# jizongFox/MI-based-Regularized-Semi-supervised-Segmentation

Measured on AMD Instinct MI355X. Metric: images/sec (UNet+IIC fwd/bwd) ACDC 256^2, higher is better.
Workload: dtype bf16; 1 GPU; udaiic train step, ACDC-shaped 1x256x256 4-class slices, LB=UB=16 per GPU, taps Conv5/Up_conv3/Up_conv2, K=20 x 5 sub-heads, paddings [1,3] (BASELINE configs[1]); mi_precision=f16f8, global_batch=32, parallelism=dp1, launch_tape=True, tape_ops=170, tape_replays_in_run=449

## Files before the change

### include/miseg_hip.h

```cpp
#ifndef MISEG_HIP_H
#define MISEG_HIP_H

#include <stdint.h>

#ifdef __cplusplus
extern "C" {
#endif

#define MISEG_F32 0
#define MISEG_BF16 1
#define MISEG_F16 2

#define MISEG_OK 0
#define MISEG_E_INVALID (-1)
#define MISEG_E_LAUNCH (-2)

int miseg_version(void);
const char* miseg_last_error(void);
int miseg_stream_wait_stream(void* waiter, void* producer);

int64_t miseg_tape_begin(void);
int miseg_tape_end(int64_t tape);
int miseg_tape_free(int64_t tape);
int64_t miseg_tape_mark(int64_t tape);
// ... 194 lines not shown
int miseg_bn_relu_fwd_acc(void* stream, int dt, const void* raw, int64_t N, int64_t H, int64_t W, int64_t C, const void* acc,
                          const float* gamma, const float* beta, float eps, float momentum, float* rmean, float* rvar, int64_t* nbt,
                          float* saved, void* y, void* pooled);
int64_t miseg_bn_bwd_ws_bytes(int64_t N, int64_t H, int64_t W, int64_t C);
int miseg_bn_relu_bwd(void* stream, int dt, const void* raw, const void* y, const void* gy, const void* gpool,
                      int64_t N, int64_t H, int64_t W, int64_t C, const float* gamma, const float* saved,
                      int training, void* graw, float* ggamma, float* gbeta, void* ws, int64_t ws_bytes);
int miseg_bn_relu_bwd_sync(void* stream, int dt, const void* raw, const void* y, const void* gy, const void* gpool,
                           int64_t N, int64_t H, int64_t W, int64_t C, const float* gamma, const float* saved,
                           int training, void* graw, float* ggamma, float* gbeta, void* ws, int64_t ws_bytes,
                           int32_t* sync_counter);
int miseg_bn_relu_bwd_dual(void* stream, int dt, const void* raw, const void* gy, const void* gpool, const void* gy2,
                           int64_t n2_begin, int64_t n2_end, int64_t N, int64_t H, int64_t W, int64_t C, const float* gamma,
                           const float* saved, int training, void* graw, float* ggamma, float* gbeta, void* ws,
                           int64_t ws_bytes);
int64_t miseg_bn_relu_bwd_acc_supported(int dt, int64_t N, int64_t H, int64_t W, int64_t C);
int miseg_bn_relu_bwd_dual_acc(void* stream, int dt, const void* raw, const void* gy, const void* gpool, const void* gy2, int64_t n2_begin,
                               int64_t n2_end, int64_t N, int64_t H, int64_t W, int64_t C, const float* gamma, const float* saved,
                               int training, void* graw, float* ggamma, float* gbeta, void* ws, int64_t ws_bytes, void* acc);
int miseg_bn_relu_bwd_ext(void* stream, int dt, const void* raw, const void* gy, int64_t N, int64_t H, int64_t W, int64_t C,
                          const float* gamma, const float* saved, int training, void* graw, float* ggamma, float* gbeta,
                          const float* ext_parts, int64_t ext_nparts, void* ws, int64_t ws_bytes);
int miseg_bn_relu_bwd_stats(void* stream, int dt, const void* raw, const void* gy, int64_t N, int64_t H, int64_t W, int64_t C,
                            const float* gamma, const float* saved, int training, float* bwd_coef, float* ggamma,
                            float* gbeta, const float* ext_parts, int64_t ext_nparts, void* ws, int64_t ws_bytes);
int64_t miseg_conv3x3_dgrad_bn_supported(int dt, int64_t K, int64_t N, int64_t H, int64_t W, int64_t Cs, int pool_out);
int64_t miseg_conv3x3_dgrad_red_parts(int dt, int64_t K, int64_t N, int64_t H, int64_t W, int64_t Cs);
int miseg_conv3x3_dgrad_bn(void* stream, int dt, const void* raw_or_graw, const void* gy, const float* bwd_coef, int64_t K,
                           int64_t N, int64_t H, int64_t W, const void* packed_w, int64_t Cs, void* out, int pool_out,
                           const void* red_raw, const float* red_saved, float* red_parts);
// ... 63 lines not shown
```

### mi-based-regularized-semi-supervised-segmentation_amd/csrc/api.hip

```cpp
#include <stdarg.h>

#include "common.h"

namespace miseg_core {
static thread_local char g_err[512] = "";
char* last_error_buf() { return g_err; }
int fail(int code, const char* fmt, ...) {
    va_list ap;
    va_start(ap, fmt);
    vsnprintf(g_err, sizeof(g_err), fmt, ap);
    va_end(ap);
    return code;
}
}

extern "C" int miseg_version(void) { return 406; }
extern "C" const char* miseg_last_error(void) { return miseg::last_error_buf(); }

namespace miseg_core {
static hipEvent_t next_fork_event() {
    constexpr int kRing = 256, kDev = 16;
    struct Ring { hipEvent_t ev[kRing]; int made = 0, next = 0; };
    static thread_local Ring rings[kDev];
    int dev = 0;
    if (hipGetDevice(&dev) != hipSuccess || dev < 0 || dev >= kDev) return nullptr;
    Ring& r = rings[dev];
    constexpr unsigned flags = hipEventDisableTiming | hipEventDisableSystemFence;
    if (r.made < kRing) {
        if (hipEventCreateWithFlags(&r.ev[r.made], flags) != hipSuccess) return nullptr;
        ++r.made;
    }
// ... 1 lines not shown
    r.next = (r.next + 1) % kRing;
    return ev;
}
}

extern "C" int miseg_stream_wait_stream(void* waiter, void* producer) {
    MISEG_TAPE(miseg_stream_wait_stream, waiter, producer);
    if (waiter == producer) return MISEG_OK;
    hipEvent_t ev = miseg_core::next_fork_event();
    if (!ev) return miseg_core::fail(MISEG_E_LAUNCH, "stream_wait_stream: hipEventCreateWithFlags failed");
    hipError_t e = hipEventRecord(ev, reinterpret_cast<hipStream_t>(producer));
    if (e == hipSuccess) e = hipStreamWaitEvent(reinterpret_cast<hipStream_t>(waiter), ev, 0);
    if (e != hipSuccess) return miseg_core::fail(MISEG_E_LAUNCH, "stream_wait_stream: %s", hipGetErrorString(e));
    return MISEG_OK;
}
```

### mi-based-regularized-semi-supervised-segmentation_amd/csrc/bn.hip

```cpp
#include "common.h"

namespace miseg {

__global__ __launch_bounds__(256) void bn_finalize_kernel(const float* __restrict__ parts, int nparts, int C, float count,
                                                          const float* __restrict__ gamma, const float* __restrict__ beta, float eps,
                                                          float momentum, float* __restrict__ rmean, float* __restrict__ rvar,
                                                          long long* __restrict__ nbt, float* __restrict__ saved) {
    __shared__ float red[17];
    const int c = blockIdx.x;
    float s1 = 0.f, s2 = 0.f;
    for (int q = threadIdx.x; q < nparts; q += 256) {
        s1 += parts[((size_t)q * 2 + 0) * C + c];
        s2 += parts[((size_t)q * 2 + 1) * C + c];
    }
    s1 = block_sum(s1, red);
    s2 = block_sum(s2, red);
    if (threadIdx.x == 0) {
        const float mean = s1 / count;
        float var = s2 / count - mean * mean;
        var = fmaxf(var, 0.f);
        const float invstd = rsqrtf(var + eps);
        const float sc = gamma[c] * invstd;
        saved[c] = mean; saved[C + c] = invstd; saved[2 * C + c] = sc; saved[3 * C + c] = beta[c] - mean * sc;
        if (rmean) {
// ... 529 lines not shown
    if (dt == MISEG_F32) {
        if (pooled) hipLaunchKernelGGL((bn_relu_fwd_kernel<float, true, true>), dim3(nb), dim3(256), 0, st, (const float*)raw, (int)N, (int)H, (int)W, (int)C, saved, (float*)y, (float*)pooled, a);
        else hipLaunchKernelGGL((bn_relu_fwd_kernel<float, false, true>), dim3(nb), dim3(256), 0, st, (const float*)raw, (int)N, (int)H, (int)W, (int)C, saved, (float*)y, (float*)nullptr, a);
    } else if (dt == MISEG_BF16) {
        if (pooled) hipLaunchKernelGGL((bn_relu_fwd_kernel<bf16, true, true>), dim3(nb), dim3(256), 0, st, (const bf16*)raw, (int)N, (int)H, (int)W, (int)C, saved, (bf16*)y, (bf16*)pooled, a);
        else hipLaunchKernelGGL((bn_relu_fwd_kernel<bf16, false, true>), dim3(nb), dim3(256), 0, st, (const bf16*)raw, (int)N, (int)H, (int)W, (int)C, saved, (bf16*)y, (bf16*)nullptr, a);
    } else return fail(MISEG_E_INVALID, "bn_relu_fwd_acc: bad dtype");
    MISEG_LAUNCH_CHECK("bn_relu_fwd_kernel");
    return MISEG_OK;
}

extern "C" int64_t miseg_bn_bwd_ws_bytes(int64_t N, int64_t H, int64_t W, int64_t C) {
    return ((int64_t)red_blocks(N * H * W, 1) * 2 * C + 3 * C) * 4;
}

static int bn_relu_bwd_impl(void* stream, int dt, const void* raw, const void* gy, const void* gpool, int64_t N, int64_t H, int64_t W, int64_t C,
                            const float* gamma, const float* saved, int training, void* graw, float* ggamma, float* gbeta, void* ws,
                            int64_t ws_bytes, int32_t* sync_counter, float* bwd_coef, const void* gy2 = nullptr, int64_t n2_begin = 0,
                            int64_t n2_end = 0, void* acc = nullptr) {
    MISEG_REQUIRE(raw && (gy || gpool) && gamma && saved && (graw || bwd_coef) && ggamma && gbeta && ws, "bn_relu_bwd: null pointer");
    MISEG_REQUIRE(!acc || (graw && !bwd_coef && !sync_counter && C <= kBnAccMaxC && ((uintptr_t)acc & 7) == 0), "bn_relu_bwd_acc: needs the apply pass, C <= 256 and an 8-byte aligned accumulator");
    MISEG_REQUIRE(!gy2 || (0 <= n2_begin && n2_begin < n2_end && n2_end <= N && (gy || gpool)), "bn_relu_bwd: bad sample range of the second gradient");
    const int V = dt == MISEG_BF16 ? 8 : 4;
    const int CV = (int)(C / V);
    MISEG_REQUIRE(C % V == 0 && 256 % CV == 0, "bn_relu_bwd: C/%d must divide 256", V);
    MISEG_REQUIRE(!gpool || (H % 2 == 0 && W % 2 == 0), "bn_relu_bwd: pooling needs even H, W");
    MISEG_REQUIRE(ws_bytes >= miseg_bn_bwd_ws_bytes(N, H, W, C), "bn_relu_bwd: workspace too small");
    hipStream_t st = as_stream(stream);
    const int64_t npix = N * H * W;
    int nb = red_blocks(npix, CV);
    if (sync_counter && C % 4 == 0 && C <= 256) nb = (int)std::max<int64_t>(1, std::min<int64_t>(nb, kFinishFloats / (2 * C)));
    float* parts = (float*)ws;
    float* coeffs = parts + (size_t)nb * 2 * C;
    const bool finish = sync_counter && C % 4 == 0 && C <= 256 && (int64_t)nb * 2 * C <= kFinishFloats;
    const size_t lb = std::max<size_t>((size_t)256 * 2 * V * 4, finish ? (size_t)(1024 + 2 * C) * 4 : 0);
    BnBwdFinish fin{finish ? reinterpret_cast<unsigned int*>(sync_counter) : nullptr, gamma, coeffs, ggamma, gbeta, (float)npix, training, bwd_coef,
                    static_cast<unsigned long long*>(acc)};
    MISEG_REQUIRE(!acc || nb <= kBnAccMaxBlocks, "bn_relu_bwd_acc: %d reduce blocks exceed the accumulator's no-wrap bound", nb);
    const int64_t p2lo = n2_begin * H * W, p2hi = n2_end * H * W;
#define RED(TT, POOL) hipLaunchKernelGGL((bn_relu_bwd_reduce_kernel<TT, POOL>), dim3(nb), dim3(256), lb, st, (const TT*)raw, (const TT*)gy, (const TT*)gpool, (int)N, (int)H, (int)W, (int)C, saved, parts, fin, BnGy2<TT>{(const TT*)gy2, p2lo, p2hi})
    if (dt == MISEG_F32) { if (gpool) RED(float, true); else RED(float, false); }
    else if (dt == MISEG_BF16) { if (gpool) RED(bf16, true); else RED(bf16, false); }
    else return fail(MISEG_E_INVALID, "bn_relu_bwd: bad dtype");
#undef RED
    MISEG_LAUNCH_CHECK("bn_relu_bwd_reduce_kernel");
    if (!finish && !acc) {
        hipLaunchKernelGGL(bn_bwd_finalize_kernel, dim3((unsigned)C), dim3(256), 0, st, parts, nb, (int)C, (float)npix, gamma, saved, training, coeffs, ggamma, gbeta, bwd_coef);
        MISEG_LAUNCH_CHECK("bn_bwd_finalize_kernel");
    }
    if (!graw) return MISEG_OK;
    const int na = ew_blocks((gpool ? npix / 4 : npix) * CV);
    const BnBwdAccArgs ba{static_cast<const unsigned long long*>(acc), gamma, ggamma, gbeta, (float)npix, training};
#define APP(TT, POOL, ACCV) hipLaunchKernelGGL((bn_bwd_apply_kernel<TT, POOL, ACCV>), dim3(na), dim3(256), 0, st, (const TT*)raw, (const TT*)gy, (const TT*)gpool, (int)N, (int)H, (int)W, (int)C, saved, coeffs, (TT*)graw, BnGy2<TT>{(const TT*)gy2, p2lo, p2hi}, ba)
    if (acc) {
        if (dt == MISEG_F32) { if (gpool) APP(float, true, true); else APP(float, false, true); }
        else { if (gpool) APP(bf16, true, true); else APP(bf16, false, true); }
    } else {
        if (dt == MISEG_F32) { if (gpool) APP(float, true, false); else APP(float, false, false); }
        else { if (gpool) APP(bf16, true, false); else APP(bf16, false, false); }
    }
#undef APP
    MISEG_LAUNCH_CHECK("bn_bwd_apply_kernel");
    return MISEG_OK;
}

extern "C" int miseg_bn_relu_bwd_sync(void* stream, int dt, const void* raw, const void* y, const void* gy, const void* gpool, int64_t N,
                                      int64_t H, int64_t W, int64_t C, const float* gamma, const float* saved, int training, void* graw,
                                      float* ggamma, float* gbeta, void* ws, int64_t ws_bytes, int32_t* sync_counter) {
    MISEG_TAPE(miseg_bn_relu_bwd_sync, stream, dt, raw, y, gy, gpool, N, H, W, C, gamma, saved, training, graw, ggamma, gbeta, ws, ws_bytes, sync_counter);
    MISEG_F16_DISPATCH_ON(dt, miseg_bn_relu_bwd_sync, stream, MISEG_BF16, raw, y, gy, gpool, N, H, W, C, gamma, saved, training, graw, ggamma, gbeta, ws,
                          ws_bytes, sync_counter);
    (void)y;
    MISEG_REQUIRE(graw, "bn_relu_bwd: null pointer");
    return bn_relu_bwd_impl(stream, dt, raw, gy, gpool, N, H, W, C, gamma, saved, training, graw, ggamma, gbeta, ws, ws_bytes, sync_counter, nullptr);
}

extern "C" int miseg_bn_relu_bwd_dual(void* stream, int dt, const void* raw, const void* gy, const void* gpool, const void* gy2, int64_t n2_begin,
                                      int64_t n2_end, int64_t N, int64_t H, int64_t W, int64_t C, const float* gamma, const float* saved, int training,
                                      void* graw, float* ggamma, float* gbeta, void* ws, int64_t ws_bytes) {
    MISEG_TAPE(miseg_bn_relu_bwd_dual, stream, dt, raw, gy, gpool, gy2, n2_begin, n2_end, N, H, W, C, gamma, saved, training, graw, ggamma, gbeta, ws, ws_bytes);
    MISEG_F16_DISPATCH_ON(dt, miseg_bn_relu_bwd_dual, stream, MISEG_BF16, raw, gy, gpool, gy2, n2_begin, n2_end, N, H, W, C, gamma, saved, training, graw,
                          ggamma, gbeta, ws, ws_bytes);
    MISEG_REQUIRE(graw, "bn_relu_bwd_dual: null pointer");
    return bn_relu_bwd_impl(stream, dt, raw, gy, gpool, N, H, W, C, gamma, saved, training, graw, ggamma, gbeta, ws, ws_bytes, nullptr, nullptr, gy2, n2_begin, n2_end);
}

extern "C" int miseg_bn_relu_bwd_dual_acc(void* stream, int dt, const void* raw, const void* gy, const void* gpool, const void* gy2, int64_t n2_begin,
                                          int64_t n2_end, int64_t N, int64_t H, int64_t W, int64_t C, const float* gamma, const float* saved,
                                          int training, void* graw, float* ggamma, float* gbeta, void* ws, int64_t ws_bytes, void* acc) {
    MISEG_TAPE(miseg_bn_relu_bwd_dual_acc, stream, dt, raw, gy, gpool, gy2, n2_begin, n2_end, N, H, W, C, gamma, saved, training, graw, ggamma, gbeta, ws, ws_bytes, acc);
    MISEG_F16_DISPATCH_ON(dt, miseg_bn_relu_bwd_dual_acc, stream, MISEG_BF16, raw, gy, gpool, gy2, n2_begin, n2_end, N, H, W, C, gamma, saved, training, graw,
                          ggamma, gbeta, ws, ws_bytes, acc);
    MISEG_REQUIRE(graw && acc, "bn_relu_bwd_dual_acc: null pointer");
    return bn_relu_bwd_impl(stream, dt, raw, gy, gpool, N, H, W, C, gamma, saved, training, graw, ggamma, gbeta, ws, ws_bytes, nullptr, nullptr, gy2, n2_begin, n2_end, acc);
}

extern "C" int64_t miseg_bn_relu_bwd_acc_supported(int dt, int64_t N, int64_t H, int64_t W, int64_t C) {
    const int V = (dt == MISEG_F32) ? 4 : 8;
    if (C % V || C > kBnAccMaxC || 256 % (C / V)) return 0;
// ... 138 lines not shown
```

### mi-based-regularized-semi-supervised-segmentation_amd/csrc/conv.hip

```cpp
#include "common.h"

namespace miseg {

constexpr int kCT = 256;
constexpr int TH = 16;
constexpr int CK = 32;

template <typename T> struct Mma;
template <> struct Mma<bf16> {
    static constexpr int CKP = 40;
    static constexpr int KP = 48;
    static constexpr int VEC = 8;
    typedef s16x8 Frag;
    static __device__ __forceinline__ Frag load(const bf16* base, int kq) { return *reinterpret_cast<const Frag*>(base + 8 * kq); }
    static __device__ __forceinline__ void mma_chunk(const Frag& a, const Frag& b, f32x4& c) {
        c = __builtin_amdgcn_mfma_f32_16x16x32_bf16(a, b, c, 0, 0, 0);
    }
};
template <> struct Mma<float> {
    static constexpr int CKP = 34;
    static constexpr int KP = 34;
    static constexpr int VEC = 4;
    struct Frag { float v[8]; };
    static __device__ __forceinline__ Frag load(const float* base, int kq) {
// ... 1714 lines not shown
    constexpr bool kFusable = !DU && (NV == 2 || NV == 4);
    if constexpr (kFusable) {
        constexpr int FRW = fused_rw<COT, NV, POOL>();
        if constexpr (POOL) { if (bl.gy) GO(true, false, FRW) else GO(false, false, 4) }
        else { if (bl.gy && br.raw) GO(true, true, FRW) else if (bl.gy) GO(true, false, FRW) else if (br.raw) GO(false, true, FRW) else GO(false, false, 4) }
    } else {
        if (bl.gy || br.raw) return fail(MISEG_E_INVALID, "conv3x3: BatchNorm loader / reduce not built for this streaming shape");
        GO(false, false, 4)
    }
#undef GO
    return MISEG_OK;
}

static int conv3x3_fwd_impl(void* stream, int dt, const void* in0, int64_t C0, int ups0, const void* in1, int64_t C1, int ups1,
                            int64_t N, int64_t H, int64_t W, const void* packed_w, int64_t Cout, void* out, float* stats, BnFinish fin,
                            bool pool_out = false, BnLoad bl = BnLoad{nullptr, nullptr}, BnRed br = BnRed{nullptr, nullptr, nullptr}) {
    MISEG_REQUIRE(in0 && packed_w && out, "conv3x3_fwd: null pointer");
    MISEG_REQUIRE(N > 0 && H > 0 && W > 0 && Cout > 0 && C0 > 0 && C1 >= 0, "conv3x3_fwd: bad shape");
    MISEG_REQUIRE(C1 == 0 || in1, "conv3x3_fwd: second source missing");
    MISEG_REQUIRE((ups0 == 0 || ups0 == 1) && (ups1 == 0 || ups1 == 1), "conv3x3_fwd: ups must be 0/1");
    MISEG_REQUIRE((!ups0 || (H % 2 == 0 && W % 2 == 0)) && (!ups1 || (H % 2 == 0 && W % 2 == 0)), "conv3x3_fwd: upsampled size must be even");
    const int vec = dt == MISEG_BF16 ? 8 : 4;
    MISEG_REQUIRE(C0 % vec == 0 && C1 % vec == 0, "conv3x3_fwd: channel counts must be multiples of %d (use conv_small for the stem)", vec);
    ConvSrc s{in0, in1, (int)C0, (int)C1, ups0, ups1};
    const int tw = tile_w(W);
    const int th = conv_streams(dt, C0 + C1, N, H, W) ? TH : generic_tile_h(dt, H, W);
    const unsigned gx = (unsigned)(N * cdiv(H, th) * cdiv(W, tw));
    hipStream_t st = as_stream(stream);
    MISEG_REQUIRE(!bl.gy || (bl.coef && C1 == 0 && ups0 == 0), "conv3x3: the BatchNorm loader reads one full-resolution source");
    MISEG_REQUIRE(!br.raw || (br.saved && br.parts && !pool_out && !stats && Cout % 4 == 0), "conv3x3: epilogue reduce needs a full-resolution "
                  "output with a multiple of 4 channels and no forward statistics");
#define LAUNCH_TH(TT, COT, TWW, THH)                                                                                       \
    launch_tiled<TT, COT, TWW, THH, false>(dim3(gx, (unsigned)cdiv(Cout, COT)), st, s, (int)N, (int)H, (int)W, packed_w, (int)Cout, out, stats, fin, bl, br);
#define LAUNCH(TT, COT, TWW) { if (th == 8) LAUNCH_TH(TT, COT, TWW, 8) else LAUNCH_TH(TT, COT, TWW, 16) }
    MISEG_REQUIRE(!pool_out || (sumpool_supported(dt, C0 + C1, N, H, W, Cout) && C1 == 0 && !stats),
                  "conv3x3_fwd_sumpool: shape not supported (ask miseg_conv3x3_fwd_sumpool_supported)");
    if (conv_streams(dt, C0 + C1, N, H, W)) {
        int rc = MISEG_OK;
#define SLAUNCH(COT, NV, DU)                                                                                               \
    {                                                                                                                     \
        const unsigned g = (unsigned)stream_blocks(N, H, W);                                                               \
        if (pool_out && !DU) rc = launch_stream<COT, NV, false, true>(g, st, s, (int)N, (int)H, (int)W, packed_w, (int)Cout, out, stats, fin, bl, br); \
        else rc = launch_stream<COT, NV, DU, false>(g, st, s, (int)N, (int)H, (int)W, packed_w, (int)Cout, out, stats, fin, bl, br); \
    }
#define SLAUNCH_NV(COT)                                                                                                    \
    {                                                                                                                     \
        if (C1 > 0) { switch ((C0 + C1) / 8) { case 2: SLAUNCH(COT, 2, true) break; case 3: SLAUNCH(COT, 3, true) break; default: SLAUNCH(COT, 4, true) break; } } \
        else { switch (C0 / 8) { case 1: SLAUNCH(COT, 1, false) break; case 2: SLAUNCH(COT, 2, false) break; case 3: SLAUNCH(COT, 3, false) break; default: SLAUNCH(COT, 4, false) break; } } \
    }
        if (Cout <= 16) SLAUNCH_NV(16)
        else SLAUNCH_NV(32)
#undef SLAUNCH_NV
// ... 51 lines not shown
    return conv3x3_fwd_impl(stream, dt, in, Cin, 0, nullptr, 0, 0, N, H, W, packed_w, Cout, inout_pooled, nullptr, opt, true);
}

extern "C" int miseg_conv3x3_dgrad_dual(void* stream, int dt, const void* graw, int64_t K, int64_t N, int64_t H, int64_t W, const void* packed_w,
                                        int64_t C0, void* out0, int64_t C1, void* out1) {
    MISEG_TAPE(miseg_conv3x3_dgrad_dual, stream, dt, graw, K, N, H, W, packed_w, C0, out0, C1, out1);
    MISEG_F16_DISPATCH_ON(dt, miseg_conv3x3_dgrad_dual, stream, MISEG_BF16, graw, K, N, H, W, packed_w, C0, out0, C1, out1);
    MISEG_REQUIRE(out0 && out1 && C0 > 0 && C1 > 0 && C0 % 16 == 0 && C1 % 4 == 0, "conv3x3_dgrad_dual: the first source must have a multiple of "
                  "16 channels, the second a multiple of 4");
    BnFinish opt{};
    opt.out1 = out1;
    opt.split = (int)C0;
    return conv3x3_fwd_impl(stream, dt, graw, K, 0, nullptr, 0, 0, N, H, W, packed_w, C0 + C1, out0, nullptr, opt);
}

static bool dgrad_bn_stream_ok(int dt, int64_t K, int64_t N, int64_t H, int64_t W) {
    return !conv_streams(dt, K, N, H, W) || K == 16 || K == 32;
}
extern "C" int64_t miseg_conv3x3_dgrad_bn_supported(int dt, int64_t K, int64_t N, int64_t H, int64_t W, int64_t Cs, int pool_out) {
    if (dt == MISEG_F16) dt = MISEG_BF16;
    const int vec = dt == MISEG_BF16 ? 8 : 4;
    if (K % vec || !dgrad_bn_stream_ok(dt, K, N, H, W)) return 0;
    return pool_out ? sumpool_supported(dt, K, N, H, W, Cs) : 1;
}
extern "C" int64_t miseg_conv3x3_dgrad_red_parts(int dt, int64_t K, int64_t N, int64_t H, int64_t W, int64_t Cs) {
    if (dt == MISEG_F16) dt = MISEG_BF16;
    if (Cs % 4 || !dgrad_bn_stream_ok(dt, K, N, H, W)) return 0;
    return miseg_conv3x3_stats_parts(dt, K, N, H, W);
}
extern "C" int miseg_conv3x3_dgrad_bn(void* stream, int dt, const void* raw_or_graw, const void* gy, const float* bwd_coef, int64_t K,
// ... 221 lines not shown
```

### mi-based-regularized-semi-supervised-segmentation_amd/miseg_amd/tape.py

```python
from __future__ import annotations

import ctypes
import os
import warnings
from typing import List, Optional

import torch
from torch import Tensor
from torch.utils._python_dispatch import TorchDispatchMode

from . import _cabi, stepio

_HARMLESS = {
    "aten::empty.memory_format", "aten::empty_strided", "aten::empty_like", "aten::new_empty", "aten::new_empty_strided",
    "aten::view", "aten::_unsafe_view", "aten::as_strided", "aten::narrow", "aten::slice.Tensor", "aten::select.int", "aten::detach",
    "aten::alias", "aten::t", "aten::transpose.int", "aten::permute", "aten::squeeze", "aten::squeeze.dim", "aten::squeeze.dims",
    "aten::unsqueeze", "aten::expand", "aten::_reshape_alias", "aten::unbind.int", "aten::split.Tensor", "aten::split_with_sizes",
    "aten::unsafe_split.Tensor", "aten::record_stream", "aten::is_pinned", "aten::lift_fresh", "aten::view.dtype",
    "aten::is_same_size", "aten::result_type.Tensor", "aten::unfold", "aten::diagonal", "aten::chunk", "aten::reshape", "aten::flatten.using_ints",
    "aten::sym_size.int", "aten::sym_stride.int", "aten::sym_numel", "aten::sym_storage_offset", "aten::is_contiguous",
    "aten::is_contiguous.memory_format", "aten::stride.int", "aten::size.int", "aten::dim", "aten::numel", "aten::_local_scalar_dense_cpu",
    "prim::device", "prim::dtype", "prim::layout", "aten::is_non_overlapping_and_dense", "aten::sym_is_contiguous",
}

# ... 81 lines not shown
    def __del__(self):
        self.release()

    def release(self) -> None:
        if self.handle:
            try:
                _cabi.lib().miseg_tape_free(self.handle)
            except Exception:
                pass
            self.handle = 0
        self.pool = None

    def _key(self, io, li: Tensor, lt: Tensor, ui: Tensor, n_masks: int):
        from . import ops, unet_ops
        return (tuple(li.shape), tuple(lt.shape), tuple(ui.shape), li.dtype, lt.dtype, ui.dtype, li.is_contiguous(), lt.is_contiguous(),
                ui.is_contiguous(), n_masks, ops._stream(), ops._mi_precision, id(io), unet_ops.PACK_CACHE.generation,
                self.ep._model.training, self.ep._tape_signature(), id(getattr(self.ep, "_reducer", None)))

    _PERSISTENT = 4

    def step(self, io, li: Tensor, lt: Tensor, ui: Tensor, flip_masks):
        ep = self.ep
        if self.disabled is not None:
            return ep._run_step(io, li, lt, ui, flip_masks)
        key = self._key(io, li, lt, ui, len(flip_masks))
        if self.handle and key == self.key:
            return self._replay(io, li, lt, ui, flip_masks)
        if self.handle:
            if key[-self._PERSISTENT:] != self.key[-self._PERSISTENT:]:
                self.release()
                self.seen = 0
            return ep._run_step(io, li, lt, ui, flip_masks)
        if self.seen < self.warmup or not (li.is_contiguous() and lt.is_contiguous() and ui.is_contiguous()):
            self.seen += 1
# ... 122 lines not shown
```

### mi-based-regularized-semi-supervised-segmentation_amd/miseg_amd/unet_ops.py

```python
from __future__ import annotations

import os

from typing import Optional, Tuple

import struct
import weakref

import torch
from torch import Tensor

from ._cabi import call, query
from .gradslot import grad_slot
from .ops import _DT, _need_gpu, _ptr, _stream, _ws, as_nhwc, empty_nhwc, wait_stream
from .tape import keep
from . import stepio

BN_EPS, BN_MOMENTUM = 1e-5, 0.1

_WGRAD_SIDE = os.environ.get("MISEG_WGRAD_STREAM", "1") != "0"
_GRAPH_STREAMS = os.environ.get("MISEG_GRAPH_STREAMS", "1") == "1"
_wgrad_streams: dict = {}
_wgrad_dirty: set = set()

# ... 10 lines not shown
        cur = torch.cuda.current_stream(dev)
        if cur != _wgrad_streams[dev]:
            wait_stream(cur, _wgrad_streams[dev])
            _wgrad_dirty.discard(dev)


_FUSE_UPS_DGRAD = True
_DUAL_DGRAD = True
_FUSE_BN_BWD = os.environ.get("MISEG_BN_FUSE", "0") == "1"
_FUSE_BN_RED = True
_RED_ONLY = os.environ.get("MISEG_BN_RED", "0") == "1" and not _FUSE_BN_BWD
_STEM_KERNELS = os.environ.get("MISEG_STEM_KERNELS", "1") != "0"
_STEM_MAX_W = 1022
_BN_ACC = os.environ.get("MISEG_BN_ACC", "1") != "0"
_BN_ACC_BWD = os.environ.get("MISEG_BN_ACC_BWD", "0") == "1"


class _BnRec:
    __slots__ = ("raw", "saved", "shape", "parts", "nparts", "for_grad", "for_version")

    def __init__(self):
        self.raw = self.saved = self.shape = self.parts = self.for_grad = None
        self.nparts = self.for_version = 0

    def offer(self, grad: Tensor, parts: Tensor, nparts: int) -> None:
        self.parts, self.nparts, self.for_grad, self.for_version = parts, nparts, grad, grad._version

    def take(self, grad: Optional[Tensor]):
        parts, nparts, mine = self.parts, self.nparts, self.for_grad is grad and grad is not None and grad._version == self.for_version
        self.parts = self.for_grad = None
# ... 278 lines not shown
            return _ConvBNReLU._backward_fused(ctx, gy, ext_parts, ext_nparts)
        gy = None if gy is None else as_nhwc(gy.to(dtype))
        gpool = None if gpool is None else as_nhwc(gpool.to(dtype))
        graw = empty_nhwc(n, cout, h, w, dtype, dev)
        pw, pg, pb = ctx.param_refs
        ggamma, gbeta = grad_slot(pg), grad_slot(pb)
        if ggamma is None:
            ggamma = torch.empty(cout, dtype=torch.float32, device=dev)
        if gbeta is None:
            gbeta = torch.empty(cout, dtype=torch.float32, device=dev)
        ws = _ws(query("miseg_bn_bwd_ws_bytes", n, h, w, cout), dev)
        bacc = None
        if _BN_ACC_BWD and not SYNC_COUNTERS.enabled and query("miseg_bn_relu_bwd_acc_supported", _DT[dtype], n, h, w, cout):
            io = stepio.current()
            bacc = io.acc64(4 * cout + 2) if io is not None else torch.zeros(4 * cout + 2, dtype=torch.int64, device=dev)
        if ext_parts is not None and not extras and gpool is None and gy is not None and not want_pool and dtype != torch.float16:
            call("miseg_bn_relu_bwd_ext", _stream(), _DT[dtype], _ptr(raw), _ptr(gy), n, h, w, cout, _ptr(gamma), _ptr(saved), int(training),
                 _ptr(graw), _ptr(ggamma), _ptr(gbeta), _ptr(ext_parts), ext_nparts, _ptr(ws), ws.numel(),
                 work=(0.0, float(raw.element_size()) * n * h * w * cout * 3.0), tag=f"bn_relu_bwd[{h}x{w},{cout}]")
        elif bacc is not None:
            g2, n0, n1 = (as_nhwc(extra[0]), extra[1], extra[2]) if extra is not None else (None, 0, 0)
            call("miseg_bn_relu_bwd_dual_acc", _stream(), _DT[dtype], _ptr(raw), _ptr(gy), _ptr(gpool), _ptr(g2), n0, n1, n, h, w, cout, _ptr(gamma),
                 _ptr(saved), int(training), _ptr(graw), _ptr(ggamma), _ptr(gbeta), _ptr(ws), ws.numel(), _ptr(bacc),
                 work=(0.0, float(raw.element_size()) * n * h * w * cout * 5.0), tag=f"bn_relu_bwd[{h}x{w},{cout}]")
        elif extra is not None:
            g2, n0, n1, _ = extra
            g2 = as_nhwc(g2)
            call("miseg_bn_relu_bwd_dual", _stream(), _DT[dtype], _ptr(raw), _ptr(gy), _ptr(gpool), _ptr(g2), n0, n1, n, h, w, cout, _ptr(gamma),
                 _ptr(saved), int(training), _ptr(graw), _ptr(ggamma), _ptr(gbeta), _ptr(ws), ws.numel(),
                 work=(0.0, float(raw.element_size()) * n * h * w * cout * 5.0), tag=f"bn_relu_bwd[{h}x{w},{cout}]")
        else:
            call("miseg_bn_relu_bwd_sync", _stream(), _DT[dtype], _ptr(raw), _ptr(y), _ptr(gy), _ptr(gpool), n, h, w, cout, _ptr(gamma), _ptr(saved),
                 int(training), _ptr(graw), _ptr(ggamma), _ptr(gbeta), _ptr(ws), ws.numel(), _ptr(SYNC_COUNTERS.take(dev)),
                 work=(0.0, float(raw.element_size()) * n * h * w * cout * 5.0), tag=f"bn_relu_bwd[{h}x{w},{cout}]")
        gw = None
        if ctx.needs_input_grad[2]:
            gw = grad_slot(pw)
            side = None
            if gw is None:
                gw = torch.empty_like(weight)
            elif _WGRAD_SIDE and (_GRAPH_STREAMS or not torch.cuda.is_current_stream_capturing()):
                side = wgrad_stream(dev)
            cur = torch.cuda.current_stream(dev)
            if side is not None:
                if not _wgrad_dirty:
                    torch.autograd.Variable._execution_engine.queue_callback(join_wgrad_streams)
                wait_stream(side, cur)
                for t in (graw, x0, x1, getattr(ctx, "image", None)):
                    keep(t, side)
                _wgrad_dirty.add(dev)
            stem_wg = bool(ctx.stem and not _FUSE_BN_BWD)
            ws2 = _ws(query("miseg_conv3x3_stem_wgrad_ws_bytes", cout) if stem_wg else query("miseg_conv3x3_wgrad_ws_bytes", n, h, w, c0 + c1, cout), dev)
            gw_full = gw if (weight.shape[1] == c0 + c1 or stem_wg) else torch.empty((cout, c0 + c1, 3, 3), dtype=torch.float32, device=dev)
            if side is not None:
                keep(ws2, side)
                if gw_full is not gw:
                    keep(gw_full, side)

            def launch(stream_handle):
                if stem_wg:
                    img = ctx.image
                    call("miseg_conv3x3_stem_wgrad", stream_handle, _DT[dtype], _ptr(img if img is not None else x0), int(img is not None),
# ... 1 lines not shown
                         work=(18.0 * cout * n * h * w, float(raw.element_size()) * n * h * w * (c0 + cout)), tag=f"conv3x3_wgrad[{h}x{w},{c0 + c1}->{cout}]")
                    return
                call("miseg_conv3x3_wgrad", stream_handle, _DT[dtype], _ptr(x0), c0, ups0, _ptr(x1), c1, ups1, n, h, w, _ptr(graw), cout, _ptr(gw_full),
                     _ptr(ws2), ws2.numel(), work=(18.0 * (c0 + c1) * cout * n * h * w, float(raw.element_size()) * n * h * w * (c0 + c1 + cout)),
                     tag=f"conv3x3_wgrad[{h}x{w},{c0 + c1}->{cout}]")
                if gw_full is not gw:
                    call("miseg_conv3x3_wgrad_slice", stream_handle, _ptr(gw_full), cout, c0 + c1, weight.shape[1], _ptr(gw))
            from . import _cabi
            if side is None:
                launch(_stream())
            elif _cabi.TIMER is not None:
                with torch.cuda.stream(side):
                    launch(_stream())
            else:
                launch(side.cuda_stream)
        grads = [None, None]
        from .ops import _GradJoin
        if _DUAL_DGRAD and x1 is not None and ctx.needs_input_grad[0] and ctx.needs_input_grad[1] and not ups0 and not ups1 and \
                c0 % 16 == 0 and c1 % 4 == 0 and not _GradJoin.enabled and not (_FUSE_BN_BWD and _FUSE_BN_RED) and not _RED_ONLY:
            packed = _pack(weight, dtype, 1, 0, c0 + c1)
            g0, g1 = empty_nhwc(n, c0, h, w, dtype, dev), empty_nhwc(n, c1, h, w, dtype, dev)
            call("miseg_conv3x3_dgrad_dual", _stream(), _DT[dtype], _ptr(graw), cout, n, h, w, _ptr(packed), c0, _ptr(g0), c1, _ptr(g1),
                 work=(18.0 * (c0 + c1) * cout * n * h * w, float(raw.element_size()) * n * h * w * (c0 + c1 + cout)),
                 tag=f"conv3x3_dgrad[{h}x{w},{cout}->{c0}+{c1}]")
            return g0, g1, gw, ggamma, gbeta, None, None, None, None, None, None, None, None, None, None, None
        for s, (cb, cs, ups, xs) in enumerate(((0, c0, ups0, x0), (c0, c1, ups1, x1))):
            if xs is None or not ctx.needs_input_grad[s]:
                continue
            packed = _pack(weight, dtype, 1, cb, cs)
            if ups and _FUSE_UPS_DGRAD and query("miseg_conv3x3_fwd_sumpool_supported", _DT[dtype], cout, n, h, w, cs):
# ... 224 lines not shown
```

Measured before the change: 4942 images/s.

## Split BN-ReLU backward apply and dgrad into image-chunk waves

Splits the BatchNorm+ReLU backward into a reduce pass and a per-image-range apply pass. It then interleaves apply and conv dgrad over chunks of images so each chunk's dgrad reads graw while it is still cache-resident. The wgrad side stream is signalled after the last apply chunk rather than before the whole backward. It is enabled by default for large layers above a byte threshold. It adds more, smaller kernel launches and gives up some wgrad overlap, since wgrad now waits until all applies have finished.

```diff
diff --git a/include/miseg_hip.h b/include/miseg_hip.h
--- a/include/miseg_hip.h
+++ b/include/miseg_hip.h
@@ -232,6 +232,20 @@
                            int64_t n2_begin, int64_t n2_end, int64_t N, int64_t H, int64_t W, int64_t C, const float* gamma,
                            const float* saved, int training, void* graw, float* ggamma, float* gbeta, void* ws,
                            int64_t ws_bytes);
+int miseg_bn_relu_bwd_reduce(void* stream, int dt, const void* raw, const void* gy, const void* gpool, const void* gy2,
+                             int64_t n2_begin, int64_t n2_end, int64_t N, int64_t H, int64_t W, int64_t C, const float* gamma,
+                             const float* saved, int training, float* ggamma, float* gbeta, void* ws, int64_t ws_bytes);
+int miseg_bn_relu_bwd_apply(void* stream, int dt, const void* raw, const void* gy, const void* gpool, const void* gy2,
+                            int64_t n2_begin, int64_t n2_end, int64_t N, int64_t H, int64_t W, int64_t C, const float* saved,
+                            const void* ws, int64_t ws_bytes, int64_t n_lo, int64_t n_hi, void* graw);
+int miseg_conv3x3_dgrad_range(void* stream, int dt, const void* grad_out, int64_t K, int64_t N, int64_t H, int64_t W,
+                              const void* packed_w, int64_t C0, void* out0, int64_t C1, void* out1, int mode, int64_t n_lo,
+                              int64_t n_hi);
+int miseg_conv_bn_relu_bwd_waves(void* stream, void* side, int dt, const void* raw, const void* gy, const void* gpool,
+                                 const void* gy2, int64_t n2_begin, int64_t n2_end, int64_t N, int64_t H, int64_t W, int64_t K,
+                                 const float* gamma, const float* saved, int training, void* graw, float* ggamma, float* gbeta,
+                                 void* ws, int64_t ws_bytes, int dgrad_mode, const void* packed_w, int64_t C0, void* out0,
+                                 int64_t C1, void* out1, int64_t chunk, int first_to_last);
 int64_t miseg_bn_relu_bwd_acc_supported(int dt, int64_t N, int64_t H, int64_t W, int64_t C);
 int miseg_bn_relu_bwd_dual_acc(void* stream, int dt, const void* raw, const void* gy, const void* gpool, const void* gy2, int64_t n2_begin,
                                int64_t n2_end, int64_t N, int64_t H, int64_t W, int64_t C, const float* gamma, const float* saved,
diff --git a/mi-based-regularized-semi-supervised-segmentation_amd/csrc/api.hip b/mi-based-regularized-semi-supervised-segmentation_amd/csrc/api.hip
--- a/mi-based-regularized-semi-supervised-segmentation_amd/csrc/api.hip
+++ b/mi-based-regularized-semi-supervised-segmentation_amd/csrc/api.hip
@@ -14,7 +14,7 @@
 }
 }
 
-extern "C" int miseg_version(void) { return 406; }
+extern "C" int miseg_version(void) { return 407; }
 extern "C" const char* miseg_last_error(void) { return miseg::last_error_buf(); }
 
 namespace miseg_core {
@@ -46,3 +46,31 @@
     if (e != hipSuccess) return miseg_core::fail(MISEG_E_LAUNCH, "stream_wait_stream: %s", hipGetErrorString(e));
     return MISEG_OK;
 }
+
+extern "C" int miseg_conv_bn_relu_bwd_waves(void* stream, void* side, int dt, const void* raw, const void* gy, const void* gpool, const void* gy2,
+                                            int64_t n2_begin, int64_t n2_end, int64_t N, int64_t H, int64_t W, int64_t K, const float* gamma,
+                                            const float* saved, int training, void* graw, float* ggamma, float* gbeta, void* ws, int64_t ws_bytes,
+                                            int dgrad_mode, const void* packed_w, int64_t C0, void* out0, int64_t C1, void* out1, int64_t chunk,
+                                            int first_to_last) {
+    MISEG_TAPE(miseg_conv_bn_relu_bwd_waves, stream, side, dt, raw, gy, gpool, gy2, n2_begin, n2_end, N, H, W, K, gamma, saved, training, graw, ggamma, gbeta,
+               ws, ws_bytes, dgrad_mode, packed_w, C0, out0, C1, out1, chunk, first_to_last);
+    MISEG_REQUIRE(N > 0 && chunk > 0 && dgrad_mode >= -1 && dgrad_mode <= 3 && graw, "conv_bn_relu_bwd_waves: bad args");
+    int rc = miseg_bn_relu_bwd_reduce(stream, dt, raw, gy, gpool, gy2, n2_begin, n2_end, N, H, W, K, gamma, saved, training, ggamma, gbeta, ws, ws_bytes);
+    if (rc != MISEG_OK) return rc;
+    const int64_t nchunks = (N + chunk - 1) / chunk;
+    for (int64_t i = 0; i < nchunks; ++i) {
+        const int64_t c = first_to_last ? i : nchunks - 1 - i;
+        const int64_t n_lo = c * chunk, n_hi = n_lo + chunk < N ? n_lo + chunk : N;
+        rc = miseg_bn_relu_bwd_apply(stream, dt, raw, gy, gpool, gy2, n2_begin, n2_end, N, H, W, K, saved, ws, ws_bytes, n_lo, n_hi, graw);
+        if (rc != MISEG_OK) return rc;
+        if (i == nchunks - 1 && side) {
+            rc = miseg_stream_wait_stream(side, stream);
+            if (rc != MISEG_OK) return rc;
+        }
+        if (dgrad_mode >= 0) {
+            rc = miseg_conv3x3_dgrad_range(stream, dt, graw, K, N, H, W, packed_w, C0, out0, C1, out1, dgrad_mode, n_lo, n_hi);
+            if (rc != MISEG_OK) return rc;
+        }
+    }
+    return MISEG_OK;
+}
diff --git a/mi-based-regularized-semi-supervised-segmentation_amd/csrc/bn.hip b/mi-based-regularized-semi-supervised-segmentation_amd/csrc/bn.hip
--- a/mi-based-regularized-semi-supervised-segmentation_amd/csrc/bn.hip
+++ b/mi-based-regularized-semi-supervised-segmentation_amd/csrc/bn.hip
@@ -567,11 +567,40 @@
     return ((int64_t)red_blocks(N * H * W, 1) * 2 * C + 3 * C) * 4;
 }
 
+static int bn_bwd_apply_range(hipStream_t st, int dt, const void* raw, const void* gy, const void* gpool, int64_t N, int64_t H, int64_t W, int64_t C,
+                              const float* gamma, const float* saved, const float* coeffs, int training, void* graw, float* ggamma, float* gbeta,
+                              const void* gy2, int64_t n2_begin, int64_t n2_end, void* acc, int64_t n_lo, int64_t n_hi) {
+    MISEG_REQUIRE(0 <= n_lo && n_lo < n_hi && n_hi <= N, "bn_relu_bwd_apply: bad image range");
+    const int V = dt == MISEG_BF16 ? 8 : 4;
+    const int CV = (int)(C / V);
+    const size_t es = dt == MISEG_BF16 ? 2 : 4;
+    const int64_t npix = N * H * W, nc = n_hi - n_lo, cpix = nc * H * W;
+    const size_t off = (size_t)n_lo * H * W * C * es, offp = (size_t)n_lo * (H / 2) * (W / 2) * C * es;
+    const char* raw_c = (const char*)raw + off;
+    const char* gy_c = gy ? (const char*)gy + off : nullptr;
+    const char* gp_c = gpool ? (const char*)gpool + offp : nullptr;
+    char* graw_c = (char*)graw + off;
+    const int64_t p2lo = (n2_begin - n_lo) * H * W, p2hi = (n2_end - n_lo) * H * W;
+    const int na = ew_blocks((gpool ? cpix / 4 : cpix) * CV);
+    const BnBwdAccArgs ba{static_cast<const unsigned long long*>(acc), gamma, ggamma, gbeta, (float)npix, training};
+#define APP(TT, POOL, ACCV) hipLaunchKernelGGL((bn_bwd_apply_kernel<TT, POOL, ACCV>), dim3(na), dim3(256), 0, st, (const TT*)raw_c, (const TT*)gy_c, (const TT*)gp_c, (int)nc, (int)H, (int)W, (int)C, saved, coeffs, (TT*)graw_c, BnGy2<TT>{(const TT*)gy2, p2lo, p2hi}, ba)
+    if (acc) {
+        if (dt == MISEG_F32) { if (gpool) APP(float, true, true); else APP(float, false, true); }
+        else { if (gpool) APP(bf16, true, true); else APP(bf16, false, true); }
+    } else {
+        if (dt == MISEG_F32) { if (gpool) APP(float, true, false); else APP(float, false, false); }
+        else { if (gpool) APP(bf16, true, false); else APP(bf16, false, false); }
+    }
+#undef APP
+    MISEG_LAUNCH_CHECK("bn_bwd_apply_kernel");
+    return MISEG_OK;
+}
+
 static int bn_relu_bwd_impl(void* stream, int dt, const void* raw, const void* gy, const void* gpool, int64_t N, int64_t H, int64_t W, int64_t C,
                             const float* gamma, const float* saved, int training, void* graw, float* ggamma, float* gbeta, void* ws,
                             int64_t ws_bytes, int32_t* sync_counter, float* bwd_coef, const void* gy2 = nullptr, int64_t n2_begin = 0,
-                            int64_t n2_end = 0, void* acc = nullptr) {
-    MISEG_REQUIRE(raw && (gy || gpool) && gamma && saved && (graw || bwd_coef) && ggamma && gbeta && ws, "bn_relu_bwd: null pointer");
+                            int64_t n2_end = 0, void* acc = nullptr, bool stats_only = false) {
+    MISEG_REQUIRE(raw && (gy || gpool) && gamma && saved && (graw || bwd_coef || stats_only) && ggamma && gbeta && ws, "bn_relu_bwd: null pointer");
     MISEG_REQUIRE(!acc || (graw && !bwd_coef && !sync_counter && C <= kBnAccMaxC && ((uintptr_t)acc & 7) == 0), "bn_relu_bwd_acc: needs the apply pass, C <= 256 and an 8-byte aligned accumulator");
     MISEG_REQUIRE(!gy2 || (0 <= n2_begin && n2_begin < n2_end && n2_end <= N && (gy || gpool)), "bn_relu_bwd: bad sample range of the second gradient");
     const int V = dt == MISEG_BF16 ? 8 : 4;
@@ -602,19 +631,7 @@
         MISEG_LAUNCH_CHECK("bn_bwd_finalize_kernel");
     }
     if (!graw) return MISEG_OK;
-    const int na = ew_blocks((gpool ? npix / 4 : npix) * CV);
-    const BnBwdAccArgs ba{static_cast<const unsigned long long*>(acc), gamma, ggamma, gbeta, (float)npix, training};
-#define APP(TT, POOL, ACCV) hipLaunchKernelGGL((bn_bwd_apply_kernel<TT, POOL, ACCV>), dim3(na), dim3(256), 0, st, (const TT*)raw, (const TT*)gy, (const TT*)gpool, (int)N, (int)H, (int)W, (int)C, saved, coeffs, (TT*)graw, BnGy2<TT>{(const TT*)gy2, p2lo, p2hi}, ba)
-    if (acc) {
-        if (dt == MISEG_F32) { if (gpool) APP(float, true, true); else APP(float, false, true); }
-        else { if (gpool) APP(bf16, true, true); else APP(bf16, false, true); }
-    } else {
-        if (dt == MISEG_F32) { if (gpool) APP(float, true, false); else APP(float, false, false); }
-        else { if (gpool) APP(bf16, true, false); else APP(bf16, false, false); }
-    }
-#undef APP
-    MISEG_LAUNCH_CHECK("bn_bwd_apply_kernel");
-    return MISEG_OK;
+    return bn_bwd_apply_range(st, dt, raw, gy, gpool, N, H, W, C, gamma, saved, coeffs, training, graw, ggamma, gbeta, gy2, n2_begin, n2_end, acc, 0, N);
 }
 
 extern "C" int miseg_bn_relu_bwd_sync(void* stream, int dt, const void* raw, const void* y, const void* gy, const void* gpool, int64_t N,
@@ -636,6 +653,32 @@
                           ggamma, gbeta, ws, ws_bytes);
     MISEG_REQUIRE(graw, "bn_relu_bwd_dual: null pointer");
     return bn_relu_bwd_impl(stream, dt, raw, gy, gpool, N, H, W, C, gamma, saved, training, graw, ggamma, gbeta, ws, ws_bytes, nullptr, nullptr, gy2, n2_begin, n2_end);
+}
+
+extern "C" int miseg_bn_relu_bwd_reduce(void* stream, int dt, const void* raw, const void* gy, const void* gpool, const void* gy2, int64_t n2_begin,
+                                        int64_t n2_end, int64_t N, int64_t H, int64_t W, int64_t C, const float* gamma, const float* saved,
+                                        int training, float* ggamma, float* gbeta, void* ws, int64_t ws_bytes) {
+    MISEG_TAPE(miseg_bn_relu_bwd_reduce, stream, dt, raw, gy, gpool, gy2, n2_begin, n2_end, N, H, W, C, gamma, saved, training, ggamma, gbeta, ws, ws_bytes);
+    MISEG_F16_DISPATCH_ON(dt, miseg_bn_relu_bwd_reduce, stream, MISEG_BF16, raw, gy, gpool, gy2, n2_begin, n2_end, N, H, W, C, gamma, saved, training, ggamma,
+                          gbeta, ws, ws_bytes);
+    return bn_relu_bwd_impl(stream, dt, raw, gy, gpool, N, H, W, C, gamma, saved, training, nullptr, ggamma, gbeta, ws, ws_bytes, nullptr, nullptr, gy2, n2_begin,
+                            n2_end, nullptr, true);
+}
+
+extern "C" int miseg_bn_relu_bwd_apply(void* stream, int dt, const void* raw, const void* gy, const void* gpool, const void* gy2, int64_t n2_begin,
+                                       int64_t n2_end, int64_t N, int64_t H, int64_t W, int64_t C, const float* saved, const void* ws, int64_t ws_bytes,
+                                       int64_t n_lo, int64_t n_hi, void* graw) {
+    MISEG_TAPE(miseg_bn_relu_bwd_apply, stream, dt, raw, gy, gpool, gy2, n2_begin, n2_end, N, H, W, C, saved, ws, ws_bytes, n_lo, n_hi, graw);
+    MISEG_F16_DISPATCH_ON(dt, miseg_bn_relu_bwd_apply, stream, MISEG_BF16, raw, gy, gpool, gy2, n2_begin, n2_end, N, H, W, C, saved, ws, ws_bytes, n_lo, n_hi, graw);
+    MISEG_REQUIRE(raw && (gy || gpool) && saved && ws && graw && (dt == MISEG_F32 || dt == MISEG_BF16), "bn_relu_bwd_apply: bad args");
+    MISEG_REQUIRE(!gy2 || (0 <= n2_begin && n2_begin < n2_end && n2_end <= N), "bn_relu_bwd_apply: bad sample range of the second gradient");
+    const int V = dt == MISEG_BF16 ? 8 : 4;
+    MISEG_REQUIRE(C % V == 0 && 256 % (C / V) == 0, "bn_relu_bwd_apply: C/%d must divide 256", V);
+    MISEG_REQUIRE(!gpool || (H % 2 == 0 && W % 2 == 0), "bn_relu_bwd_apply: pooling needs even H, W");
+    MISEG_REQUIRE(ws_bytes >= miseg_bn_bwd_ws_bytes(N, H, W, C), "bn_relu_bwd_apply: workspace too small");
+    const float* coeffs = (const float*)ws + (size_t)red_blocks(N * H * W, (int)(C / V)) * 2 * C;
+    return bn_bwd_apply_range(as_stream(stream), dt, raw, gy, gpool, N, H, W, C, nullptr, saved, coeffs, 0, graw, nullptr, nullptr, gy2, n2_begin, n2_end,
+                              nullptr, n_lo, n_hi);
 }
 
 extern "C" int miseg_bn_relu_bwd_dual_acc(void* stream, int dt, const void* raw, const void* gy, const void* gpool, const void* gy2, int64_t n2_begin,
diff --git a/mi-based-regularized-semi-supervised-segmentation_amd/csrc/conv.hip b/mi-based-regularized-semi-supervised-segmentation_amd/csrc/conv.hip
--- a/mi-based-regularized-semi-supervised-segmentation_amd/csrc/conv.hip
+++ b/mi-based-regularized-semi-supervised-segmentation_amd/csrc/conv.hip
@@ -1752,7 +1752,9 @@
 
 static int conv3x3_fwd_impl(void* stream, int dt, const void* in0, int64_t C0, int ups0, const void* in1, int64_t C1, int ups1,
                             int64_t N, int64_t H, int64_t W, const void* packed_w, int64_t Cout, void* out, float* stats, BnFinish fin,
-                            bool pool_out = false, BnLoad bl = BnLoad{nullptr, nullptr}, BnRed br = BnRed{nullptr, nullptr, nullptr}) {
+                            bool pool_out = false, BnLoad bl = BnLoad{nullptr, nullptr}, BnRed br = BnRed{nullptr, nullptr, nullptr},
+                            int64_t Nsel = 0) {
+    if (Nsel <= 0) Nsel = N;
     MISEG_REQUIRE(in0 && packed_w && out, "conv3x3_fwd: null pointer");
     MISEG_REQUIRE(N > 0 && H > 0 && W > 0 && Cout > 0 && C0 > 0 && C1 >= 0, "conv3x3_fwd: bad shape");
     MISEG_REQUIRE(C1 == 0 || in1, "conv3x3_fwd: second source missing");
@@ -1762,7 +1764,7 @@
     MISEG_REQUIRE(C0 % vec == 0 && C1 % vec == 0, "conv3x3_fwd: channel counts must be multiples of %d (use conv_small for the stem)", vec);
     ConvSrc s{in0, in1, (int)C0, (int)C1, ups0, ups1};
     const int tw = tile_w(W);
-    const int th = conv_streams(dt, C0 + C1, N, H, W) ? TH : generic_tile_h(dt, H, W);
+    const int th = conv_streams(dt, C0 + C1, Nsel, H, W) ? TH : generic_tile_h(dt, H, W);
     const unsigned gx = (unsigned)(N * cdiv(H, th) * cdiv(W, tw));
     hipStream_t st = as_stream(stream);
     MISEG_REQUIRE(!bl.gy || (bl.coef && C1 == 0 && ups0 == 0), "conv3x3: the BatchNorm loader reads one full-resolution source");
@@ -1771,9 +1773,9 @@
 #define LAUNCH_TH(TT, COT, TWW, THH)                                                                                       \
     launch_tiled<TT, COT, TWW, THH, false>(dim3(gx, (unsigned)cdiv(Cout, COT)), st, s, (int)N, (int)H, (int)W, packed_w, (int)Cout, out, stats, fin, bl, br);
 #define LAUNCH(TT, COT, TWW) { if (th == 8) LAUNCH_TH(TT, COT, TWW, 8) else LAUNCH_TH(TT, COT, TWW, 16) }
-    MISEG_REQUIRE(!pool_out || (sumpool_supported(dt, C0 + C1, N, H, W, Cout) && C1 == 0 && !stats),
+    MISEG_REQUIRE(!pool_out || (sumpool_supported(dt, C0 + C1, Nsel, H, W, Cout) && C1 == 0 && !stats),
                   "conv3x3_fwd_sumpool: shape not supported (ask miseg_conv3x3_fwd_sumpool_supported)");
-    if (conv_streams(dt, C0 + C1, N, H, W)) {
+    if (conv_streams(dt, C0 + C1, Nsel, H, W)) {
         int rc = MISEG_OK;
 #define SLAUNCH(COT, NV, DU)                                                                                               \
     {                                                                                                                     \
@@ -1855,6 +1857,34 @@
     return conv3x3_fwd_impl(stream, dt, graw, K, 0, nullptr, 0, 0, N, H, W, packed_w, C0 + C1, out0, nullptr, opt);
 }
 
+extern "C" int miseg_conv3x3_dgrad_range(void* stream, int dt, const void* graw, int64_t K, int64_t N, int64_t H, int64_t W, const void* packed_w,
+                                         int64_t C0, void* out0, int64_t C1, void* out1, int mode, int64_t n_lo, int64_t n_hi) {
+    MISEG_TAPE(miseg_conv3x3_dgrad_range, stream, dt, graw, K, N, H, W, packed_w, C0, out0, C1, out1, mode, n_lo, n_hi);
+    MISEG_F16_DISPATCH_ON(dt, miseg_conv3x3_dgrad_range, stream, MISEG_BF16, graw, K, N, H, W, packed_w, C0, out0, C1, out1, mode, n_lo, n_hi);
+    MISEG_REQUIRE(graw && out0 && 0 <= n_lo && n_lo < n_hi && n_hi <= N && mode >= 0 && mode <= 3 && (dt == MISEG_F32 || dt == MISEG_BF16),
+                  "conv3x3_dgrad_range: bad args");
+    const size_t es = dt == MISEG_BF16 ? 2 : 4;
+    const bool pool = mode >= 2;
+    MISEG_REQUIRE(!pool || (H % 2 == 0 && W % 2 == 0), "conv3x3_dgrad_range: pooled output needs even H, W");
+    const size_t pix_in = (size_t)n_lo * H * W, pix_out = pool ? (size_t)n_lo * (H / 2) * (W / 2) : pix_in;
+    const void* in = (const char*)graw + pix_in * K * es;
+    void* o0 = (char*)out0 + pix_out * C0 * es;
+    BnFinish opt{};
+    int64_t Cout = C0;
+    if (mode == 1) {
+        MISEG_REQUIRE(out1 && C0 > 0 && C1 > 0 && C0 % 16 == 0 && C1 % 4 == 0, "conv3x3_dgrad_range: the first source must have a multiple of 16 "
+                      "channels, the second a multiple of 4");
+        opt.out1 = (char*)out1 + pix_out * C1 * es;
+        opt.split = (int)C0;
+        Cout = C0 + C1;
+    } else if (mode == 3) {
+        MISEG_REQUIRE(miseg_conv3x3_fwd_sumpool_acc_supported(dt, K, N, H, W), "conv3x3_dgrad_range: the adding pooled form serves streaming shapes only");
+        opt.accumulate_out = 1;
+    }
+    return conv3x3_fwd_impl(stream, dt, in, K, 0, nullptr, 0, 0, n_hi - n_lo, H, W, packed_w, Cout, o0, nullptr, opt, pool, BnLoad{nullptr, nullptr},
+                            BnRed{nullptr, nullptr, nullptr}, N);
+}
+
 static bool dgrad_bn_stream_ok(int dt, int64_t K, int64_t N, int64_t H, int64_t W) {
     return !conv_streams(dt, K, N, H, W) || K == 16 || K == 32;
 }
diff --git a/mi-based-regularized-semi-supervised-segmentation_amd/miseg_amd/tape.py b/mi-based-regularized-semi-supervised-segmentation_amd/miseg_amd/tape.py
--- a/mi-based-regularized-semi-supervised-segmentation_amd/miseg_amd/tape.py
+++ b/mi-based-regularized-semi-supervised-segmentation_amd/miseg_amd/tape.py
@@ -119,10 +119,10 @@
     def _key(self, io, li: Tensor, lt: Tensor, ui: Tensor, n_masks: int):
         from . import ops, unet_ops
         return (tuple(li.shape), tuple(lt.shape), tuple(ui.shape), li.dtype, lt.dtype, ui.dtype, li.is_contiguous(), lt.is_contiguous(),
-                ui.is_contiguous(), n_masks, ops._stream(), ops._mi_precision, id(io), unet_ops.PACK_CACHE.generation,
+                ui.is_contiguous(), n_masks, ops._stream(), ops._mi_precision, id(io), unet_ops.waves_config(), unet_ops.PACK_CACHE.generation,
                 self.ep._model.training, self.ep._tape_signature(), id(getattr(self.ep, "_reducer", None)))
 
-    _PERSISTENT = 4
+    _PERSISTENT = 5
 
     def step(self, io, li: Tensor, lt: Tensor, ui: Tensor, flip_masks):
         ep = self.ep
diff --git a/mi-based-regularized-semi-supervised-segmentation_amd/miseg_amd/unet_ops.py b/mi-based-regularized-semi-supervised-segmentation_amd/miseg_amd/unet_ops.py
--- a/mi-based-regularized-semi-supervised-segmentation_amd/miseg_amd/unet_ops.py
+++ b/mi-based-regularized-semi-supervised-segmentation_amd/miseg_amd/unet_ops.py
@@ -48,6 +48,35 @@
 _STEM_MAX_W = 1022
 _BN_ACC = os.environ.get("MISEG_BN_ACC", "1") != "0"
 _BN_ACC_BWD = os.environ.get("MISEG_BN_ACC_BWD", "0") == "1"
+_BWD_WAVES = os.environ.get("MISEG_BWD_WAVES", "1") != "0"
+_WAVES_MIN_BYTES = int(os.environ.get("MISEG_BWD_WAVES_MIN_BYTES", 256 << 20))
+_WAVES_CHUNK = int(os.environ.get("MISEG_BWD_WAVES_CHUNK", 16))
+_WAVES_FIRST_TO_LAST = os.environ.get("MISEG_BWD_WAVES_ORDER", "last") == "first"
+
+
+def waves_config() -> tuple:
+    return (_BWD_WAVES, _WAVES_MIN_BYTES, _WAVES_CHUNK, _WAVES_FIRST_TO_LAST)
+
+
+def _waves_mode(ctx, dtype, gpool, ext_parts, bacc) -> Optional[int]:
+    from . import ops
+    from .ops import _GradJoin
+    training, ups0, ups1, want_pool, c0, c1, n, h, w, cout = ctx.cfg
+    if not ops._LIB_FORK or torch.cuda.is_current_stream_capturing():
+        return None
+    if not _BWD_WAVES or dtype not in (torch.bfloat16, torch.float16) or ext_parts is not None or bacc is not None or SYNC_COUNTERS.enabled \
+            or _FUSE_BN_BWD or _RED_ONLY or _GradJoin.enabled or n <= _WAVES_CHUNK or 3 * 2 * n * h * w * cout <= _WAVES_MIN_BYTES:
+        return None
+    need0, need1 = ctx.needs_input_grad[0], ctx.needs_input_grad[1] and c1 > 0
+    if not need0 and not need1:
+        return -1
+    if c1 == 0 and need0:
+        if ups0:
+            return 2 if _FUSE_UPS_DGRAD and query("miseg_conv3x3_fwd_sumpool_supported", _DT[dtype], cout, n, h, w, c0) else None
+        return 0
+    if _DUAL_DGRAD and need0 and need1 and not ups0 and not ups1 and c0 % 16 == 0 and c1 % 4 == 0:
+        return 1
+    return None
 
 
 class _BnRec:
@@ -356,7 +385,34 @@
         if _BN_ACC_BWD and not SYNC_COUNTERS.enabled and query("miseg_bn_relu_bwd_acc_supported", _DT[dtype], n, h, w, cout):
             io = stepio.current()
             bacc = io.acc64(4 * cout + 2) if io is not None else torch.zeros(4 * cout + 2, dtype=torch.int64, device=dev)
-        if ext_parts is not None and not extras and gpool is None and gy is not None and not want_pool and dtype != torch.float16:
+        gw, side = None, None
+        if ctx.needs_input_grad[2]:
+            gw = grad_slot(pw)
+            if gw is None:
+                gw = torch.empty_like(weight)
+            elif _WGRAD_SIDE and (_GRAPH_STREAMS or not torch.cuda.is_current_stream_capturing()):
+                side = wgrad_stream(dev)
+        use_ext = ext_parts is not None and not extras and gpool is None and gy is not None and not want_pool and dtype != torch.float16
+        wmode = _waves_mode(ctx, dtype, gpool, ext_parts if use_ext else None, bacc)
+        wgrads = None
+        if wmode is not None:
+            g2, n0, n1 = (as_nhwc(extra[0]), extra[1], extra[2]) if extra is not None else (None, 0, 0)
+            wg0 = wg1 = packed = None
+            if wmode == 1:
+                packed = _pack(weight, dtype, 1, 0, c0 + c1)
+                wg0, wg1 = empty_nhwc(n, c0, h, w, dtype, dev), empty_nhwc(n, c1, h, w, dtype, dev)
+            elif wmode >= 0:
+                packed = _pack(weight, dtype, 1, 0, c0)
+                wg0 = empty_nhwc(n, c0, h >> ups0, w >> ups0, dtype, dev)
+            es = raw.element_size()
+            cd = c0 + (c1 if wmode == 1 else 0)
+            call("miseg_conv_bn_relu_bwd_waves", _stream(), side.cuda_stream if side is not None else None, _DT[dtype], _ptr(raw), _ptr(gy), _ptr(gpool),
+                 _ptr(g2), n0, n1, n, h, w, cout, _ptr(gamma), _ptr(saved), int(training), _ptr(graw), _ptr(ggamma), _ptr(gbeta), _ptr(ws), ws.numel(),
+                 wmode, _ptr(packed), c0, _ptr(wg0), c1 if wmode == 1 else 0, _ptr(wg1), _WAVES_CHUNK, int(_WAVES_FIRST_TO_LAST),
+                 work=(18.0 * cd * cout * n * h * w if wmode >= 0 else 0.0, float(es) * n * h * w * (5.0 * cout + (cout + cd / (4 ** ups0) if wmode >= 0 else 0))),
+                 tag=f"bn_relu_bwd+dgrad_waves[{h}x{w},{cout}->{cd if wmode >= 0 else 0}]")
+            wgrads = (wg0, wg1)
+        elif use_ext:
             call("miseg_bn_relu_bwd_ext", _stream(), _DT[dtype], _ptr(raw), _ptr(gy), n, h, w, cout, _ptr(gamma), _ptr(saved), int(training),
                  _ptr(graw), _ptr(ggamma), _ptr(gbeta), _ptr(ext_parts), ext_nparts, _ptr(ws), ws.numel(),
                  work=(0.0, float(raw.element_size()) * n * h * w * cout * 3.0), tag=f"bn_relu_bwd[{h}x{w},{cout}]")
@@ -375,19 +431,13 @@
             call("miseg_bn_relu_bwd_sync", _stream(), _DT[dtype], _ptr(raw), _ptr(y), _ptr(gy), _ptr(gpool), n, h, w, cout, _ptr(gamma), _ptr(saved),
                  int(training), _ptr(graw), _ptr(ggamma), _ptr(gbeta), _ptr(ws), ws.numel(), _ptr(SYNC_COUNTERS.take(dev)),
                  work=(0.0, float(raw.element_size()) * n * h * w * cout * 5.0), tag=f"bn_relu_bwd[{h}x{w},{cout}]")
-        gw = None
         if ctx.needs_input_grad[2]:
-            gw = grad_slot(pw)
-            side = None
-            if gw is None:
-                gw = torch.empty_like(weight)
-            elif _WGRAD_SIDE and (_GRAPH_STREAMS or not torch.cuda.is_current_stream_capturing()):
-                side = wgrad_stream(dev)
             cur = torch.cuda.current_stream(dev)
             if side is not None:
                 if not _wgrad_dirty:
                     torch.autograd.Variable._execution_engine.queue_callback(join_wgrad_streams)
-                wait_stream(side, cur)
+                if wmode is None:
+                    wait_stream(side, cur)
                 for t in (graw, x0, x1, getattr(ctx, "image", None)):
                     keep(t, side)
                 _wgrad_dirty.add(dev)
@@ -419,6 +469,8 @@
                     launch(_stream())
             else:
                 launch(side.cuda_stream)
+        if wgrads is not None:
+            return wgrads[0], wgrads[1], gw, ggamma, gbeta, None, None, None, None, None, None, None, None, None, None, None
         grads = [None, None]
         from .ops import _GradJoin
         if _DUAL_DGRAD and x1 is not None and ctx.needs_input_grad[0] and ctx.needs_input_grad[1] and not ups0 and not ups1 and \
```

Measured after the change: 4792 images/s. 0.97x the previous value.
